# monoamine11231/Example-GUI-OpenCL-Raytracer

Hardware: AMD Instinct MI355X
Metric: Mrays/s at 1920x1080 depth 4, aggregate over n_gpus; rays = path segments + shadow rays as the reference casts them (value_traced: only those the kernel really traces) (higher is better)
Workload: dtype f32; 1 GPU; C2: scenes/render.map (regenerated), camera raypng.c:17-21, 1920x1080, depth 4, 2 soft-shadow samples, 4x256^2 textures + 4096x3072 skybox (procedural); frame=1920x1080, arithmetic=fast

## Files before the change

### example_gui_opencl_raytracer_amd/csrc/hip_wrap.cpp

```cpp
#include <hip/hip_runtime.h>

#include <algorithm>
#include <cstdarg>
#include <cstdint>
#include <cstdio>
#include <cstdlib>
#include <cmath>
#include <cstring>
#include <string>
#include <vector>

#include "../../include/hip_wrap_ext.h"
#include "png_codec.h"
#include "scene_prep.h"
#include "whitted_params.h"

extern "C" hipError_t wt_fast_launch_trace(const whitted_params*, int, unsigned, size_t, hipStream_t);
extern "C" hipError_t wt_fast_launch_raygen(const raygen_params*, hipStream_t);
extern "C" hipError_t wt_strict_launch_trace(const whitted_params*, int, unsigned, size_t, hipStream_t);
extern "C" hipError_t wt_strict_launch_raygen(const raygen_params*, hipStream_t);
extern "C" hipError_t wt_fast_launch_unit(int, const float*, float*, unsigned, unsigned, unsigned, unsigned, hipStream_t);
extern "C" hipError_t wt_strict_launch_unit(int, const float*, float*, unsigned, unsigned, unsigned, unsigned, hipStream_t);
extern "C" hipError_t wt_fast_launch_unit_scene(const whitted_params*, int, int, const float*, float*, unsigned, unsigned, unsigned, size_t, hipStream_t);
extern "C" hipError_t wt_strict_launch_unit_scene(const whitted_params*, int, int, const float*, float*, unsigned, unsigned, unsigned, size_t, hipStream_t);
// ... 364 lines not shown
            HIP_OK(hipMalloc((void**)&I->d_grid_box, bx.size() * 4), "Couldn't allocate device memory");
            HIP_OK(hipMemcpy(I->d_grid_start, st.data(), st.size() * 4, hipMemcpyHostToDevice), "Couldn't transfer the data from host to the device");
            HIP_OK(hipMemcpy(I->d_grid_items, it.data(), it.size() * 4, hipMemcpyHostToDevice), "Couldn't transfer the data from host to the device");
            HIP_OK(hipMemcpy(I->d_grid_box, bx.data(), bx.size() * 4, hipMemcpyHostToDevice), "Couldn't transfer the data from host to the device");
            std::vector<float> cg(4 * it.size(), 0.0f);
            for (size_t k = 0; k < pairs; k++) memcpy(&cg[4 * k], &geom[4 * (size_t)it[k]], 16);
            HIP_OK(hipMalloc((void**)&I->d_grid_geom, cg.size() * 4), "Couldn't allocate device memory");
            HIP_OK(hipMemcpy(I->d_grid_geom, cg.data(), cg.size() * 4, hipMemcpyHostToDevice), "Couldn't transfer the data from host to the device");
            I->grid_ok = true;
        }
    }
    I->geom_f4 = f4;
    I->scene_generation++;
    I->prep_s = s; I->prep_p = p; I->prep_l = l; I->prep_ns = ns; I->prep_np = np; I->prep_nl = nl;
}

Buffer* buffer_arg(cl_wrap* w, cl_uint kernel_id, cl_uint arg) {
    if (!is_registered(w, kernel_id, arg)) die("Couldn't run the kernel");
    return (Buffer*)w->buffers[kernel_id][arg];
}

void bind_scene(cl_wrap* w, Impl* I, cl_uint kid, whitted_params& P, int& flags, size_t& dyn_lds) {
    Kernel& k = I->kernels[kid];
    Buffer* bs = buffer_arg(w, kid, 1);
    Buffer* bp = buffer_arg(w, kid, 2);
    Buffer* bl = buffer_arg(w, kid, 3);
    uint32_t ns = read_count(k, 4), np = read_count(k, 5), nl = read_count(k, 6);
    Buffer* tex = buffer_arg(w, kid, 8);
    Buffer* sky = buffer_arg(w, kid, 9);
    if (!tex->image || !sky->image) die("Couldn't run the kernel");
    prepare_scene(I, bs, ns, bp, np, bl, nl);
    ensure_allocated(I, bs); ensure_allocated(I, bp);
    P.geom = I->d_geom; P.ptex = I->d_ptex; P.geom_f4 = (uint32_t)I->geom_f4;
    P.lpt = (I->have_lpt && !(I->variant & 128)) ? 1u : 0u;
    P.vis = (I->strict && ns <= VIS_MAX_SPHERES && (np == 0 || P.lpt) && !(I->variant & 256)) ? ((I->variant & 1024) ? 2u : 1u) : 0u;
    P.spheres_raw = (const uint8_t*)bs->dptr; P.planes_raw = (const uint8_t*)bp->dptr;
    P.ns = ns; P.np = np; P.nl = nl;
    P.through = I->through;
    P.tex = (const uint32_t*)tex->dptr; P.tex_w = (int)tex->w; P.tex_h = (int)tex->h; P.tex_layers = (int)tex->layers;
    P.sky = (const uint32_t*)sky->dptr; P.sky_w = (int)sky->w; P.sky_h = (int)sky->h;
    if (I->grid_ok && I->use_grid && !(I->variant & 8)) {
        flags |= F_GRID;
        P.grid_pair = I->grid_pair ? 1u : 0u;
        P.grid_start = I->d_grid_start; P.grid_items = I->d_grid_items; P.grid_box = I->d_grid_box; P.grid_geom = I->d_grid_geom;
        for (int a = 0; a < 3; a++) {
            P.grid_min[a] = I->grid.gmin[a]; P.grid_inv[a] = I->grid.inv[a]; P.grid_cell[a] = I->grid.cell[a]; P.grid_res[a] = I->grid.res[a];
        }
    } else if (I->geom_f4 <= GEOM_LDS_MAX_F4 && ns <= GRID_MIN_SPHERES && !(I->variant & 1)) {
        flags |= F_GEOM_LDS;
        dyn_lds = I->geom_f4 * 16;
    }
}

struct Strip { uint32_t row0, rows; int slot; };

void run_raytracer(cl_wrap* w, Impl* I, cl_uint kid, size_t array_size, const Strip* strip = nullptr) {
    Kernel& k = I->kernels[kid];
    Buffer* rays = nullptr;
    if (is_registered(w, kid, 0)) rays = (Buffer*)w->buffers[kid][0];
    else {
        const ArgValue& v = need_value(k, 0, sizeof(cl_mem), sizeof(cl_mem));
        void* h; memcpy(&h, v.bytes, sizeof h);
        rays = lookup_handle(I, h);
        if (!rays) die("Couldn't run the kernel");
    }
    uint32_t total; memcpy(&total, need_value(k, 7, 4, 4).bytes, 4);
    Buffer* out = buffer_arg(w, kid, 10);

    uint64_t rounded = ((uint64_t)array_size + BLOCK - 1) / BLOCK * BLOCK;
    uint64_t n64 = rounded < total ? rounded : total;
    ensure_allocated(I, out);
    if (n64 > out->size / 4) n64 = out->size / 4;
    if (n64 == 0) return;
    if (n64 > 0xFFFFFFFFull) die("Couldn't run the kernel");

    whitted_params P{};
    int flags = 0;
    size_t dyn_lds = 0;
    bind_scene(w, I, kid, P, flags, dyn_lds);
    P.n_items = (uint32_t)n64;
    P.depth = I->depth;
    P.out = (uint32_t*)out->dptr;
    P.out_rgb = I->debug_rgb;
    P.diag = (I->variant & 512) ? (env_int("CLWRAP_TIMELINE_EDGES", 0) ? 255u + (uint32_t)env_int("CLWRAP_TIMELINE_EDGES", 0) : 1u + (uint32_t)env_int("CLWRAP_TIMELINE_SHIFT", 0)) : 0u;

    const bool fused = I->fuse && rays->gen_valid && !rays->exposed;
    RaygenArgs g{};
    if (fused) {
        g = rays->gen;
        if (strip) {
            g.id_offset += (uint64_t)strip->row0 * g.width;
            g.n_items = strip->rows * g.width;
            P.n_items = g.n_items;
            P.out = (uint32_t*)out->dptr + (size_t)strip->row0 * g.width;
        }
        memcpy(P.corner, g.corner, 12); memcpy(P.origin, g.origin, 12);
        memcpy(P.up, g.up, 12); memcpy(P.right, g.right, 12);
        P.w_factor = g.w_factor; P.h_factor = g.h_factor; P.width = g.width; P.height = g.height;
        P.id_offset = g.id_offset;
        P.band_stride = g.band_stride; P.band_phase = g.band_phase;
        if (P.n_items > g.n_items) P.n_items = g.n_items;
        if (P.n_items == 0) return;
        P.tiled = (g.id_offset % g.width == 0 || g.band_stride > 1) && (P.n_items % g.width == 0) && !(I->variant & 2);
        P.rows = P.n_items / g.width;
        P.row_offset = (uint32_t)(g.id_offset / g.width);
        P.unit_dirs = P.ns <= GRID_MIN_SPHERES ? 1u : 0u;
    } else {
        materialise_rays(I, rays);
        ensure_allocated(I, rays);
        if ((uint64_t)P.n_items * 64 > rays->size) die("Couldn't run the kernel");
        P.rays = (const float*)rays->dptr;
        P.id_offset = I->id_offset;
        P.width = 1; P.height = 1;
        P.unit_dirs = (rays->gen_valid && !rays->exposed && P.ns <= GRID_MIN_SPHERES) ? 1u : 0u;
        if (rays->gen_valid) {
            P.id_offset = rays->gen.id_offset; P.width = rays->gen.width; P.height = rays->gen.height;
            P.band_stride = rays->gen.band_stride; P.band_phase = rays->gen.band_phase;
        } else if (I->band_stride > 1) die("Row bands need a raygen launch");
        flags |= F_RAYS;
    }
    if (I->depth > SHALLOW_LEVELS + 1) flags |= F_DEEP;
    if (!(flags & F_GEOM_LDS)) P.vis = 0;
    if (I->counting || I->stamps || I->tpt_clock) {
        if (I->counting) flags |= F_COUNT;
        P.tpt_clock = I->tpt_clock ? 1u : 0u;
        if (!I->d_counters) {
            HIP_OK(hipMalloc((void**)&I->d_counters, COUNTER_WORDS * sizeof(unsigned long long)), "Couldn't allocate device memory");
            HIP_OK(hipMemsetAsync(I->d_counters, 0, COUNTER_WORDS * sizeof(unsigned long long), I->stream), "Couldn't allocate device memory");
        }
        P.counters = I->d_counters;
    }
    unsigned grid;
    Impl::Sched& S = I->scheds[strip ? strip->slot : 0];
    bool sched_rebuild = false;
    unsigned trows = 0, tpr = 0, per_share = 0, per_share_cap = 0, base_grid = 0;
    if (P.tiled) {
        trows = (P.rows + 7) / 8; tpr = (P.width + 7) / 8;
        per_share = ((trows + 7) / 8) * tpr;
        per_share_cap = per_share;
        grid = base_grid = 8 * per_share;
    } else {
        grid = base_grid = (P.n_items + TRACE_BLOCK - 1) / TRACE_BLOCK;
    }
    if ((flags & F_DEEP) && !I->strict && (uint64_t)base_grid >= (uint64_t)I->occ_tiles_per_depth * (unsigned)I->depth && !(I->variant & 64)) flags |= F_OCC;
    const uint64_t tpt_per_node = (I->strict ? 29u : 27u) + (I->strict ? 4u : 1u) * (uint64_t)P.nl;
    const uint64_t tpt_fixed = (25u + 36u) * 64u + (uint64_t)I->depth * 3u * 64u;
    const uint64_t tpt_nslots = 8u * (uint64_t)TPT_SLOTS_PER_XCC;
    const uint64_t tpt_slice = std::min<uint64_t>(TPT_SLICE_WORDS_MAX, ((uint64_t)I->tpt_pool_mb << 18) / tpt_nslots) & ~(uint64_t)63;
    const uint64_t tpt_cap = std::min<uint64_t>(tpt_slice > tpt_fixed ? ((tpt_slice - tpt_fixed) / tpt_per_node) & ~(uint64_t)63 : 0, 64960u);
    const bool tail_wanted = (flags & F_DEEP) && !(flags & F_OCC) && !(I->variant & 16) && I->tpt_max != 0u && tpt_cap >= TPT_MIN_CAP;
    bool split = false;
    if (P.tiled) {
        if (I->sched && !(I->variant & 4) && trows <= 0xFFFu && tpr <= 0xFFFu) {
            split = tail_wanted && !(flags & F_GRID) && I->split_min_quota != 0u && !(I->variant & 4096);
            if (split) { per_share_cap = per_share + SPLIT_EXTRA_PER_SHARE; grid = 8 * per_share_cap; }
            P.cost_sum = (tail_wanted && !(flags & F_GRID)) ? 1u : 0u;
            if (S.w != P.width || S.rows != P.rows || S.cap != per_share_cap || !S.cost[0]) {
                S.free_all();
                for (int i = 0; i < 2; i++) {
                    HIP_OK(hipMalloc((void**)&S.cost[i], (size_t)trows * tpr * 4), "Couldn't allocate device memory");
                    HIP_OK(hipMalloc((void**)&S.order[i], (size_t)grid * 4), "Couldn't allocate device memory");
                    HIP_OK(hipEventCreateWithFlags(&S.built[i], hipEventDisableTiming), "Couldn't create a timing event");
                }
                HIP_OK(hipEventCreateWithFlags(&S.traced, hipEventDisableTiming), "Couldn't create a timing event");
                S.w = P.width; S.rows = P.rows; S.cap = per_share_cap; S.wr = 0;
            }
// ... 500 lines not shown
```

### example_gui_opencl_raytracer_amd/csrc/whitted_hit.inc

```
            cost++;
            if (COUNT) {
                c_iter++;
                unsigned long long live = __builtin_amdgcn_ballot_w64(true);
                if (lane == (unsigned)__builtin_ctzll(live)) c_witer += 64u;
            }
            const rayq r = UNIT_CT ? wt_rayq<true>(o, d) : wt_rayq<false>(o, d, P.unit_dirs != 0u);

            if (COUNT) c_probe++;
            bool lit = false;
            float tl = INFINITY;
            f3 lcol = mk3(0, 0, 0);
            auto probe_chunk = [&](auto nc, const unsigned base) {
                constexpr int N = decltype(nc)::value;
                float4 l0[N]; float bq[N], Dq[N]; bool ok[N]; bool any = false;
#pragma unroll
                for (int k = 0; k < N; k++) l0[k] = wt_geom<GEOM_LDS>(P, sg, g_lgt + 2 * (base + k));
#pragma unroll
                for (int k = 0; k < N; k++) {
                    const sph_pre pre = wt_sphere_pre(r.o, l0[k]);
                    ok[k] = wt_sphere_disc(pre, r.d, r.a4, bq[k], Dq[k]);
                    any |= ok[k];
                }
                if (__builtin_amdgcn_ballot_w64(any)) {
#pragma unroll
                    for (int k = 0; k < N; k++) {
                        float t;
                        const bool hit = wt_sphere_root(bq[k], Dq[k], r.a2, t) && ok[k];
                        if (hit && !(t >= tl)) {
                            float4 l1 = wt_geom<GEOM_LDS>(P, sg, g_lgt + 2 * (base + k) + 1);
                            tl = t;
                            f3 hp = wt_madd3(d, t, o);
                            float dist = wt_sqrt(dot3(o - hp, o - hp));
                            lcol = mk3(l1.x, l1.y, l1.z) * (1 / dist * dist);
                            lit = true;
                        }
                    }
                }
            };
            for (unsigned base = 0; base < SH::nl(P); base += 4u) {
                const unsigned left = SH::nl(P) - base;
                if (left >= 4u) probe_chunk(wt_int<4>{}, base);
                else if (left == 3u) probe_chunk(wt_int<3>{}, base);
                else if (left == 2u) probe_chunk(wt_int<2>{}, base);
                else probe_chunk(wt_int<1>{}, base);
            }
            if (__builtin_amdgcn_ballot_w64(lit)) {
                if (lit) {
                    if (GRID) {
                        if (wt_grid_occluded(P, r, tl)) lit = false;
                    }
                    for (unsigned i = 0; !GRID && i < SH::ns(P); i++) {
                        float4 s = wt_geom<GEOM_LDS>(P, sg, i);
                        float t;
                        bool hit = wt_sphere(r, s, t);
                        if (hit && t <= tl && !(__float_as_uint(s.w) >> 31)) lit = false;
                    }
                    for (unsigned i = 0; i < SH::np(P); i++) {
                        float4 n = wt_geom<GEOM_LDS>(P, sg, g_pln + 2 * i);
                        float4 p0 = wt_geom<GEOM_LDS>(P, sg, g_pln + 2 * i + 1);
                        float t;
                        bool hit = wt_plane(r, n, p0, t);
                        if (hit && t <= tl) lit = false;
                    }
                }
            }
            WT_STAMP(WT_ST_PROBE);
            if (lit) {
                WT_HIT_COLOUR(lcol);
                ended = true;
            } else {
                if (COUNT) c_seg++;
                float tbest = INFINITY;
                int best = -1;
                if (GRID) {
                    best = wt_grid_nearest(P, r, tbest);
                } else {
                    for (unsigned base = 0; base < SH::ns(P); base += 4u) {
                        float4 s4[4]; float bq[4], Dq[4]; bool ok[4]; bool any = false;
#pragma unroll
                        for (int k = 0; k < 4; k++) s4[k] = wt_geom<GEOM_LDS>(P, sg, min(base + k, SH::ns(P) - 1u));
#pragma unroll
                        for (int k = 0; k < 4; k++) {
                            const sph_pre pre = wt_sphere_pre(r.o, s4[k]);
                            ok[k] = wt_sphere_disc(pre, r.d, r.a4, bq[k], Dq[k]) && (base + k < SH::ns(P));
                            any |= ok[k];
                        }
                        if (__builtin_amdgcn_ballot_w64(any)) {
#pragma unroll
                            for (int k = 0; k < 4; k++) {
                                if (__builtin_amdgcn_ballot_w64(ok[k]) == 0) continue;
                                float t;
                                const bool hit = wt_sphere_root(bq[k], Dq[k], r.a2, t) && ok[k];
                                if (hit && !(t >= tbest)) { tbest = t; best = (int)(base + k); }
                            }
                        }
                    }
                }
                for (unsigned i = 0; i < SH::np(P); i++) {
                    float4 n = wt_geom<GEOM_LDS>(P, sg, g_pln + 2 * i);
                    float4 p0 = wt_geom<GEOM_LDS>(P, sg, g_pln + 2 * i + 1);
                    float t;
                    bool hit = wt_plane(r, n, p0, t);
                    if (hit && !(t >= tbest)) { tbest = t; best = (int)(SH::ns(P) + i); }
                }
                WT_STAMP(WT_ST_NEAREST);
                if (best < 0) {
                    if (COUNT) c_sky++;
                    WT_HIT_COLOUR(wt_texel_rgb(wt_skybox_fetch(P, d)));
                    ended = true;
                } else {
                    ip = wt_madd3(d, tbest, o);
                    prim = (unsigned)best;
                    textured = false;
                    if ((unsigned)best < SH::ns(P)) {
                        float4 s = wt_geom<GEOM_LDS>(P, sg, (unsigned)best);
                        nrm = wt_normalize(ip - mk3(s.x, s.y, s.z));
                    } else {
                        unsigned pi = (unsigned)best - SH::ns(P);
                        float4 n = wt_geom<GEOM_LDS>(P, sg, g_pln + 2 * pi);
                        nrm = mk3(n.x, n.y, n.z);
                        if (n.w != 0.0f) {
                            if (COUNT) c_tex++;
                            texpx = wt_plane_texel_fetch(P, pi, ip);
                            textured = true;
                        }
                    }
                    wt_mat_set_b(m, wt_mat_f4(P, prim, 1u, SH::ns(P)));
                    {
                        const float4 a_ = wt_mat_f4(P, prim, 0u, SH::ns(P));
                        m.rgb = mk3(a_.x, a_.y, a_.z);
                        wt_mat_set_c(m, wt_mat_f4(P, prim, 2u, SH::ns(P)));
                    }
                    ip = wt_madd3(nrm, WT_EPSILON, ip);
                    cost += 3u;
                    {
                        const f3 c_ = textured ? wt_texel_rgb(texpx) : m.rgb;
                        WT_HIT_AMBIENT(c_ * f, m.ambient);
                    }
                    view = wt_normalize(o - ip);
                    ks = f * m.specular; kd = f * m.diffuse;
                    shade = true;
                }
            }
```

### example_gui_opencl_raytracer_amd/csrc/whitted_params.h

```cpp
#ifndef WHITTED_PARAMS_H
#define WHITTED_PARAMS_H
#include <stdint.h>

#define CLW_MAX_DEPTH 32
#define CLW_NUM_COUNTERS 32
#define CLW_STAMP_SHARDS 1024

typedef struct {
    float corner[3], origin[3], up[3], right[3];
    float w_factor, h_factor;
    uint32_t width, height;
    uint64_t id_offset;
    uint32_t n_items;
    uint32_t tiled;
    uint32_t rows;
    uint32_t row_offset;
    uint32_t band_stride, band_phase;
    const uint32_t* tile_order;
    uint32_t* tile_cost;
    uint32_t* tpt_pool;
    uint32_t* tpt_flags;
    const uint32_t* tpt_jump;
    uint32_t tpt_slice_words, tpt_cap, tpt_slots, tpt_max, tpt_min;
    uint32_t tpt_clock;
    uint32_t cost_sum;
    int32_t depth;
    const float* geom;
    const float* ptex;
    const uint8_t* spheres_raw;
    const uint8_t* planes_raw;
    uint32_t ns, np, nl;
    float through;
    uint32_t geom_f4;
    uint32_t unit_dirs;
    uint32_t lpt;
    uint32_t vis;
    uint32_t diag;
    const uint32_t* grid_start;
    const uint32_t* grid_items;
    const uint32_t* grid_box;
    const float* grid_geom;
    float grid_min[3], grid_inv[3], grid_cell[3];
    uint32_t grid_pair;
    int32_t grid_res[3];
    const uint32_t* tex; int32_t tex_w, tex_h, tex_layers;
    const uint32_t* sky; int32_t sky_w, sky_h;
    const float* rays;
    uint32_t* out;
    float* out_rgb;
    unsigned long long* counters;
} whitted_params;

typedef struct {
    float corner[3], origin[3], up[3], right[3];
    float w_factor, h_factor;
    uint32_t width, height;
    uint64_t id_offset;
    uint32_t n_items;
    uint32_t band_stride, band_phase;
    float* rays;
} raygen_params;

#endif
```

### example_gui_opencl_raytracer_amd/csrc/whitted_trace.inc

```

#ifndef WT_STRICT
#error "WT_STRICT must be defined (0: fast, 1: strict)"
#endif

#define WT_EPSILON 0.001f
#define WT_THROUGH 0.8f
#define WT_DEFAULT_N 1.0f
#define WT_SOFT 2
#ifndef WT_LDS_LEVELS
#if WT_STRICT
#define WT_LDS_LEVELS 3
#else
#define WT_LDS_LEVELS 2
#endif
#endif
#ifndef WT_LDS_LEVELS_DEEP
#define WT_LDS_LEVELS_DEEP 3
#endif
#ifndef WT_LDS_LEVELS_DEEP_OCC
#define WT_LDS_LEVELS_DEEP_OCC 1
#endif
#ifndef WT_MIN_WAVES
#define WT_MIN_WAVES (WT_STRICT ? 2 : 3)
#endif
// ... 898 lines not shown
    typedef wt_shape<SHF> SH;
    const bool masked = MASKED && P.ns <= 64u;
    unsigned long long todo = !masked ? 0ull : ((P.ns == 64u ? ~0ull : ((1ull << P.ns) - 1ull)) & cand);
    for (unsigned n = 0; todo != 0ull; n++) {
        const unsigned i = (unsigned)__builtin_ctzll(todo);
        todo &= todo - 1ull;
        if ((n & 3u) == 3u) {
            unsigned live = 0u;
#pragma unroll
            for (int q = 0; q < NR; q++) live |= __float_as_uint(op[q]);
            if (__builtin_amdgcn_ballot_w64(live != 0u) == 0) break;
        }
        const float4 s = wt_geom<GEOM_LDS>(P, sg, i);
        const sph_pre pre = wt_shadow_pre(ip, s);
        const float through = (__float_as_uint(s.w) >> 31) ? P.through : 0.0f;
        float bq[NR], Dq[NR];
        bool any = false;
#pragma unroll
        for (int q = 0; q < NR; q++) any |= wt_shadow_disc_g<GEOM_LDS>(pre, rd[q], a4[q], bq[q], Dq[q]);
        if (__builtin_amdgcn_ballot_w64(any)) {
#pragma unroll
            for (int q = 0; q < NR; q++) {
                float t;
                bool hit = wt_shadow_root_g<GEOM_LDS>(bq[q], Dq[q], a2[q], t) && !(Dq[q] < 0);
                if (hit && !(t >= tl[q])) op[q] = op[q] * through;
            }
        }
    }
    for (unsigned i = 0; !masked && i < SH::ns(P); i++) {
        if ((i & 3u) == 3u) {
            unsigned live = 0u;
#pragma unroll
            for (int q = 0; q < NR; q++) live |= __float_as_uint(op[q]);
            if (__builtin_amdgcn_ballot_w64(live != 0u) == 0) break;
        }
        const float4 s = wt_geom<GEOM_LDS>(P, sg, i);
        const sph_pre pre = wt_shadow_pre(ip, s);
        const float through = (__float_as_uint(s.w) >> 31) ? P.through : 0.0f;
        float bq[NR], Dq[NR];
        bool any = false;
#pragma unroll
        for (int q = 0; q < NR; q++) any |= wt_shadow_disc_g<GEOM_LDS>(pre, rd[q], a4[q], bq[q], Dq[q]);
        if (__builtin_amdgcn_ballot_w64(any)) {
#pragma unroll
            for (int q = 0; q < NR; q++) {
                float t;
                bool hit = wt_shadow_root_g<GEOM_LDS>(bq[q], Dq[q], a2[q], t) && !(Dq[q] < 0);
                if (hit && !(t >= tl[q])) op[q] = op[q] * through;
            }
        }
    }
    for (unsigned i = 0; i < SH::np(P); i++) {
        if ((i & 3u) == 0u) {
            unsigned live = 0u;
#pragma unroll
            for (int q = 0; q < NR; q++) live |= __float_as_uint(op[q]);
            if (__builtin_amdgcn_ballot_w64(live != 0u) == 0) break;
        }
        const float4 n = wt_geom<GEOM_LDS>(P, sg, g_pln + 2 * i);
        const float4 p0 = wt_geom<GEOM_LDS>(P, sg, g_pln + 2 * i + 1);
        const float num = wt_plane_pre(ip, n, p0);
        bool skip[NR / WT_SOFT];
#pragma unroll
        for (int k = 0; k < NR / WT_SOFT; k++) skip[k] = false;
        if (CULL && SH::lpt(P) && chunk != ~0u) {
            const float4 mu = wt_geom<GEOM_LDS>(P, sg, g_pln + 2 * SH::np(P) + 2 * SH::nl(P) + chunk * SH::np(P) + i);
            const float mus[3] = {mu.x, mu.y, mu.z};
            const float an = 1e-5f * fabsf(num) * mu.w;
#pragma unroll
            for (int k = 0; k < NR / WT_SOFT && k < 3; k++) {
                const bool cannot = (num * mus[k] < 0.0f) && (fabsf(mus[k]) > __builtin_fmaf(4e-6f, dlc[k], an));
                skip[k] = __builtin_amdgcn_ballot_w64(!cannot) == 0;
            }
        }
#pragma unroll
        for (int q = 0; q < NR; q++) {
            if (!skip[q / WT_SOFT]) {
                if (wt_plane_blocks(num, n, rd[q], tl[q])) op[q] = 0.0f;
            }
        }
    }
}

__device__ __forceinline__ void wt_stage_scene(const whitted_params& P, float4* s_geom, unsigned tid, unsigned nthreads) {
    for (unsigned i = tid; i < P.geom_f4; i += nthreads) s_geom[i] = ((const float4*)P.geom)[i];
    __syncthreads();
}

#include "whitted_terms.inc"

template <int FLAGS>
struct wt_cfg {
    static constexpr bool deep = (FLAGS & 2) != 0, occ = (FLAGS & 32) != 0, grid = (FLAGS & 16) != 0;
    static constexpr int lds_levels = deep ? (occ ? WT_LDS_LEVELS_DEEP_OCC : WT_LDS_LEVELS_DEEP) : WT_LDS_LEVELS;
    static constexpr int max_levels = !deep ? 3 : ((FLAGS & 64) ? 7 : ((FLAGS & 128) ? 15 : CLW_MAX_DEPTH - 1));
    static constexpr int min_waves = deep ? (occ ? WT_OCC_WAVES : WT_MIN_WAVES) : ((grid && !WT_STRICT) ? WT_GRID_SHALLOW_WAVES : WT_SHALLOW_WAVES);
};
typedef const __attribute__((address_space(4))) whitted_params* wt_kparams_t;
template <int FLAGS>
__device__ __forceinline__ void wt_trace_body(const wt_kparams_t Pk, const unsigned wg) {
    constexpr bool COUNT = (FLAGS & WT_F_COUNT) != 0;
    constexpr bool DEEP = (FLAGS & WT_F_DEEP) != 0;
    constexpr bool GEOM_LDS = (FLAGS & WT_F_GEOM_LDS) != 0;
    constexpr bool FROM_RAYS = (FLAGS & WT_F_RAYS) != 0;
    constexpr bool GRID = (FLAGS & WT_F_GRID) != 0;
    constexpr bool UNIT_CT = !WT_STRICT && GEOM_LDS && !FROM_RAYS && !GRID;
    constexpr bool CLASSES = WT_STRICT != 0 && GEOM_LDS && !GRID;

    constexpr int LDSL = wt_cfg<FLAGS>::lds_levels;
    __shared__ float s_stk[LDSL * WT_REC * WT_BLOCK];
    __shared__ unsigned short s_tpt_bs[(DEEP && !wt_cfg<FLAGS>::occ) ? WT_TPT_MAX_BATCHES + 2 : 1];
    __shared__ unsigned s_tpt_px[(DEEP && !wt_cfg<FLAGS>::occ) ? 3 * 64 : 1];
    constexpr bool SPHCULL = DEEP && !GRID && (wt_cfg<FLAGS>::occ || WT_STRICT != 0);
    __shared__ int s_cull[SPHCULL ? 8 : 1];
    extern __shared__ float4 s_geom[];

    const whitted_params& P = *(const whitted_params*)Pk;
#if WT_TIMELINE
    const unsigned long long tl_entry = __builtin_amdgcn_s_memrealtime();
#endif

    if (GEOM_LDS) wt_stage_scene(P, s_geom, threadIdx.x, WT_BLOCK);
    const float4* sg = s_geom;
#if WT_TIMELINE
    const unsigned long long tl_staged = __builtin_amdgcn_s_memrealtime();
#endif
    WT_STAMP_DECL

    const unsigned tid = threadIdx.x;
    const unsigned lane = tid & 63u;

    bool valid;
    unsigned item;
    unsigned x = 0, y = 0;
    unsigned tile = 0xFFFFFFFFu;
    unsigned part_lg = 0u, part = 0u;
    if (P.tiled) {
        const unsigned tpr = (P.width + 7u) >> 3;
        const unsigned b = wg;
        unsigned trow, tcol;
        if (P.tile_order) {
            const unsigned t = P.tile_order[b];
            tcol = t & 0xFFFu; trow = (t >> 12) & 0xFFFu;
            part_lg = (t >> 24) & 7u; part = (t >> 27) & 15u;
            tile = (t == 0xFFFFFFFFu) ? t : trow * tpr + tcol;
        } else {
            const unsigned k = b & 7u, j = b >> 3;
            trow = (j / tpr) * 8u + k;
            tcol = j % tpr;
            tile = trow * tpr + tcol;
        }
        x = tcol * 8u + (lane & 7u);
        y = trow * 8u + (lane >> 3);
        valid = (tile != 0xFFFFFFFFu) && (x < P.width) && (y < P.rows) && ((lane >> (6u - part_lg)) == part);
        item = y * P.width + x;
    } else {
        item = wg * WT_BLOCK + tid;
        valid = item < P.n_items;
        if (P.band_stride > 1u) { y = item / P.width; x = item % P.width; }
    }
#if WT_TIMELINE
    asm volatile("" :: "v"(item), "v"(x), "v"(y));
    const unsigned long long tl_mapped = __builtin_amdgcn_s_memrealtime();
#endif
    unsigned long long gid = P.id_offset + item;
    unsigned gy = y;
    if (P.band_stride > 1u) {
        gy = ((y >> 3) * P.band_stride + P.band_phase) * 8u + (y & 7u);
        gid = (unsigned long long)gy * P.width + x;
    } else if (P.tiled) {
        gy = P.row_offset + y;
    }

    constexpr int SCRL = wt_cfg<FLAGS>::max_levels - LDSL;
    float deep[SCRL > 0 ? SCRL * WT_REC : 1];

    f3 o = mk3(0, 0, 0), d = mk3(0, 0, 1), rgb = mk3(0, 0, 0);
    int depth = 0;
    if (valid) {
        if (FROM_RAYS) {
            const float4* rr = (const float4*)(P.rays + 16 * (size_t)item);
            float4 ro = rr[0], rd = rr[1], rc = rr[2];
            o = mk3(ro.x, ro.y, ro.z); d = mk3(rd.x, rd.y, rd.z); rgb = mk3(rc.x, rc.y, rc.z);
            depth = __float_as_int(rr[3].x);
        } else {
            if (P.tiled || P.band_stride > 1u) d = wt_primary_dir_xy(P.corner, P.right, P.up, P.w_factor, P.h_factor, x, gy);
            else d = wt_primary_dir(P.corner, P.right, P.up, P.w_factor, P.h_factor, (unsigned)gid, P.width);
            o = mk3(P.origin[0], P.origin[1], P.origin[2]);
        }
    }
    float n1 = WT_DEFAULT_N, f = 1.0f;
    int sp = 0;
    unsigned rng = (unsigned)gid;
    const int D = P.depth;
    bool active = valid && depth < D;

    unsigned c_seg = 0, c_shadow = 0, c_probe = 0, c_sky = 0, c_tex = 0, c_push = 0, c_iter = 0, c_witer = 0;
    unsigned c_traced = 0;
    unsigned c_known = 0, c_visbad = 0;
    unsigned c_tptrun = 0, c_tptfail = 0, c_tptnodes = 0;

    typedef wt_shape<FLAGS> SH;
    const unsigned g_pln = SH::ns(P), g_lgt = SH::ns(P) + 2 * SH::np(P);

    const unsigned long long t_begin = ((GRID || WT_COST_LIFETIME) && P.tile_cost) ? __builtin_amdgcn_s_memtime() : 0ull;
#if WT_TIMELINE
    const unsigned long long tl_begin = __builtin_amdgcn_s_memrealtime();
    unsigned long long tl_end = tl_begin;
#endif
    unsigned cost = 0;
#ifndef WT_LCH
#define WT_LCH 3
#endif
    constexpr int LCH = WT_LCH, NR = LCH * WT_SOFT;

    constexpr bool TPT = DEEP && !wt_cfg<FLAGS>::occ;
    unsigned tpt_thresh = (TPT && P.tpt_cap != 0u) ? (part_lg != 0u ? 64u : P.tpt_max) : 0u;
    WT_STAMP(WT_ST_PROLOG);
    for (;;) {
    while ((unsigned)__builtin_popcountll(__builtin_amdgcn_ballot_w64(active)) > tpt_thresh) {
        if (active) {
            WT_STAMP(WT_ST_LOOP);
            bool ended = false, shade = false;
            f3 ip, nrm, view;
            mat_t m;
            float ks, kd;
            unsigned prim, texpx;
            bool textured;
#include "whitted_hit.inc"
            WT_STAMP(WT_ST_RESOLVE);
            if (shade) {
#include "whitted_shade.inc"
#include "whitted_bounce.inc"
            WT_STAMP(WT_ST_BOUNCE);
            }
#include "whitted_pop.inc"
            WT_STAMP(WT_ST_POP);
        }
    }
    if (!TPT || __builtin_amdgcn_ballot_w64(active) == 0) break;
    {
        bool tpt_done = false;
#include "whitted_tpt.inc"
        if (tpt_done) break;
        tpt_thresh = 0u;
    }
    }
    if (P.tiled && P.tile_cost) {
        unsigned c = cost;
        if (GRID || WT_COST_LIFETIME) c = (unsigned)min((__builtin_amdgcn_s_memtime() - t_begin) >> 8, 0xFFFFFFFFull);
        else if (P.cost_sum) for (int off = 32; off > 0; off >>= 1) c += (unsigned)__shfl_xor((int)c, off);
        else for (int off = 32; off > 0; off >>= 1) c = max(c, (unsigned)__shfl_xor((int)c, off));
#if WT_TIMELINE
        if (P.diag && P.diag < 256u) c = ((unsigned)((tl_begin >> (P.diag - 1u)) & 0xFFFFull) << 16) | (unsigned)((__builtin_amdgcn_s_memrealtime() >> (P.diag - 1u)) & 0xFFFFull);
        tl_end = __builtin_amdgcn_s_memrealtime();
#endif
        if (lane == 0 && tile != 0xFFFFFFFFu && y < P.rows) {
            if (P.cost_sum && !(WT_TIMELINE && P.diag)) atomicAdd(P.tile_cost + tile, c);
            else P.tile_cost[tile] = c;
        }
    }


    if (valid) {
        if (P.out_rgb) {
            float* q = P.out_rgb + 3 * (size_t)item;
            q[0] = rgb.x; q[1] = rgb.y; q[2] = rgb.z;
        }
        float cr = fminf(fmaxf(rgb.x, 0.0f), 1.0f) * 255.0f;
        float cg = fminf(fmaxf(rgb.y, 0.0f), 1.0f) * 255.0f;
        float cb = fminf(fmaxf(rgb.z, 0.0f), 1.0f) * 255.0f;
        P.out[item] = ((unsigned)cr << 16) | ((unsigned)cg << 8) | (unsigned)cb;
    }

#ifdef WT_STAMPS
    WT_STAMP(WT_ST_LOOP);
    __syncthreads();
    if (P.counters && lane == 0) {
        unsigned long long* sh = P.counters + CLW_NUM_COUNTERS + 16u * (wg & 1023u);
        for (int k = 0; k < WT_ST_N; k++) atomicAdd(sh + k, (unsigned long long)s_st[k]);
        atomicAdd(sh + WT_ST_N, 1ull);
    }
#endif
    if (COUNT) {
        unsigned v[14] = {c_seg, c_shadow, c_probe, c_sky, c_tex, c_push, c_iter, c_witer, c_traced, c_known, c_visbad, c_tptfail, c_tptrun, c_tptnodes};
#pragma unroll
        for (int k = 0; k < 14; k++) {
            unsigned x = v[k];
            for (int off = 32; off > 0; off >>= 1) x += __shfl_xor(x, off);
            if (lane == 0 && x) atomicAdd(P.counters + (k < 10 ? k : 18 + k), (unsigned long long)x);
        }
    }
#if WT_TIMELINE
    if (P.diag >= 256u && P.tiled && P.tile_cost && lane == 0 && tile != 0xFFFFFFFFu && y < P.rows) {
        __builtin_amdgcn_s_waitcnt(0);
        if (P.diag == 256u) P.tile_cost[tile] = ((unsigned)min(tl_begin - tl_entry, 0xFFFFull) << 16) | (unsigned)min(__builtin_amdgcn_s_memrealtime() - tl_end, 0xFFFFull);
        else P.tile_cost[tile] = ((unsigned)min(tl_staged - tl_entry, 1023ull) << 22) | ((unsigned)min(tl_mapped - tl_staged, 2047ull) << 11) | (unsigned)min(tl_begin - tl_mapped, 2047ull);
    }
#endif
}
template <int FLAGS>
__global__ void __launch_bounds__(WT_BLOCK, wt_cfg<FLAGS>::min_waves) wt_trace(const whitted_params P_arg) {
    const wt_kparams_t Pk = (wt_kparams_t)__builtin_amdgcn_kernarg_segment_ptr();
    wt_trace_body<FLAGS>(Pk, blockIdx.x);
}

#define WT_RG_BLOCK 256
__global__ void __launch_bounds__(WT_RG_BLOCK) wt_raygen(const raygen_params P) {
    constexpr int RS = WT_RG_BLOCK + 1;
    __shared__ float4 s_rec[4 * RS];
    const unsigned tid = threadIdx.x;
    const size_t base = (size_t)blockIdx.x * WT_RG_BLOCK;
    const size_t item = base + tid;
    float4 r0 = make_float4(0, 0, 0, 0), r1 = r0;
    if (item < P.n_items) {
        unsigned long long gid = P.id_offset + item;
        if (P.band_stride > 1u) {
            const unsigned y = (unsigned)(item / P.width), x = (unsigned)(item % P.width);
            gid = (unsigned long long)(((y >> 3) * P.band_stride + P.band_phase) * 8u + (y & 7u)) * P.width + x;
        }
        f3 d = wt_primary_dir(P.corner, P.right, P.up, P.w_factor, P.h_factor, (unsigned)gid, P.width);
        r0 = make_float4(P.origin[0], P.origin[1], P.origin[2], 0.0f);
        r1 = make_float4(d.x, d.y, d.z, 0.0f);
    }
    s_rec[0 * RS + tid] = r0;
    s_rec[1 * RS + tid] = r1;
    s_rec[2 * RS + tid] = make_float4(0, 0, 0, 0);
    s_rec[3 * RS + tid] = make_float4(0, 0, 0, 0);
    __syncthreads();
    float4* dst = (float4*)P.rays + base * 4;
    const size_t limit = ((size_t)P.n_items - base < WT_RG_BLOCK ? (size_t)P.n_items - base : WT_RG_BLOCK) * 4;
#pragma unroll
    for (int k = 0; k < 4; k++) {
        size_t q = (size_t)k * WT_RG_BLOCK + tid;
        if (q < limit) dst[q] = s_rec[(q & 3) * RS + (q >> 2)];
    }
}

__global__ void __launch_bounds__(256) wt_sched_build(const unsigned* __restrict__ cost, unsigned* __restrict__ order,
                                                      unsigned tpr, unsigned trows, unsigned per_share, unsigned clamp_outliers,
                                                      unsigned per_share_cap, unsigned split_slots, unsigned min_quota) {
    __shared__ unsigned hist[256];
    __shared__ unsigned base[256];
    __shared__ unsigned s_max, s_cnt, s_entries;
    __shared__ unsigned long long s_sum;
    const unsigned k = blockIdx.x, tid = threadIdx.x;
    hist[tid] = 0;
    if (tid == 0) { s_max = 1u; s_cnt = 0u; s_sum = 0ull; s_entries = 0u; }
    __syncthreads();
    unsigned cnt = 0u;
    unsigned long long sum = 0ull;
    for (unsigned j = tid; j < per_share; j += 256) {
        const unsigned trow = (j / tpr) * 8u + k;
        if (trow < trows) { sum += cost[trow * tpr + (j % tpr)]; cnt++; }
    }
    atomicAdd(&s_sum, sum); atomicAdd(&s_cnt, cnt);
    __syncthreads();
    unsigned quota = 0xFFFFFFFFu;
    if (split_slots != 0u) {
        const unsigned long long q = s_sum / split_slots;
        quota = (unsigned)(q > 0x7FFFFFFFull ? 0x7FFFFFFFull : q);
        if (quota < min_quota) quota = min_quota;
        if (quota == 0u) quota = 1u;
        for (int trial = 0; trial < 24; trial++) {
            if (tid == 0) s_entries = 0u;
            __syncthreads();
            unsigned e = 0u;
            for (unsigned j = tid; j < per_share; j += 256) {
                const unsigned trow = (j / tpr) * 8u + k;
                if (trow < trows) { unsigned lg = 0u; const unsigned c = cost[trow * tpr + (j % tpr)]; while (lg < 4u && (c >> lg) > quota) lg++; e += 1u << lg; }
            }
            atomicAdd(&s_entries, e);
            __syncthreads();
// ... 43 lines not shown
    for (unsigned j = nvalid + tid; j < per_share_cap; j += 256) order[8u * j + k] = 0xFFFFFFFFu;
}

enum { WT_U_SPHERE = 0, WT_U_PLANE = 1, WT_U_REFLECT = 2, WT_U_REFRACT = 3, WT_U_SCHLICK = 4, WT_U_CUBE = 5,
       WT_U_XORSHIFT = 6, WT_U_EMOD = 7, WT_U_SINCOS = 8, WT_U_POW = 9, WT_U_NORMALIZE = 10 };
__global__ void __launch_bounds__(64) wt_unit(int op, const float* __restrict__ in, float* __restrict__ out, unsigned n,
                                              unsigned stride_in, unsigned stride_out, unsigned aux) {
    const unsigned i = blockIdx.x * 64 + threadIdx.x;
    if (i >= n) return;
    const float* a = in + (size_t)i * stride_in;
    float* r = out + (size_t)i * stride_out;
    switch (op) {
        case WT_U_SPHERE: {
            const rayq q = wt_rayq<false>(mk3(a[0], a[1], a[2]), mk3(a[3], a[4], a[5]));
            float t;
            bool hit = wt_sphere(q, make_float4(a[6], a[7], a[8], a[9] * a[9]), t);
            r[0] = hit ? 1.0f : 0.0f; r[1] = hit ? t : 0.0f;
        } break;
        case WT_U_PLANE: {
            const rayq q = wt_rayq<false>(mk3(a[0], a[1], a[2]), mk3(a[3], a[4], a[5]));
            float t;
            bool hit = wt_plane(q, make_float4(a[6], a[7], a[8], 0.0f), make_float4(a[9], a[10], a[11], 0.0f), t);
            r[0] = hit ? 1.0f : 0.0f; r[1] = hit ? t : 0.0f;
        } break;
        case WT_U_REFLECT: {
            f3 v = wt_reflect(mk3(a[0], a[1], a[2]), mk3(a[3], a[4], a[5]));
            r[0] = v.x; r[1] = v.y; r[2] = v.z;
        } break;
        case WT_U_REFRACT: {
            f3 v = mk3(0, 0, 0);
            bool ok = wt_refract(a[0], a[1], mk3(a[2], a[3], a[4]), mk3(a[5], a[6], a[7]), v);
            r[0] = ok ? 1.0f : 0.0f; r[1] = v.x; r[2] = v.y; r[3] = v.z;
        } break;
        case WT_U_SCHLICK:
            r[0] = wt_schlick(a[0], a[1], mk3(a[2], a[3], a[4]), mk3(a[5], a[6], a[7]));
            break;
        case WT_U_CUBE: {
            int u, v;
            wt_cube_uv(mk3(a[0], a[1], a[2]), aux, u, v);
            r[0] = __int_as_float(u); r[1] = __int_as_float(v);
        } break;
        case WT_U_XORSHIFT: {
            unsigned st = __float_as_uint(a[0]);
            float v = wt_xorshift(st);
            r[0] = __uint_as_float(st); r[1] = v;
        } break;
        case WT_U_EMOD:
            r[0] = __int_as_float(wt_emod(__float_as_int(a[0]), __float_as_int(a[1])));
            break;
        case WT_U_SINCOS: {
            float sn, cs;
            if (aux) wt_sincos_angle<true>(a[0], sn, cs); else wt_sincos_angle<false>(a[0], sn, cs);
            r[0] = sn; r[1] = cs;
        } break;
        case WT_U_POW:
            r[0] = wt_pow(a[0], a[1]);
            break;
        case WT_U_NORMALIZE: {
            float len;
            f3 v = wt_normalize_len(mk3(a[0], a[1], a[2]), len);
            r[0] = v.x; r[1] = v.y; r[2] = v.z; r[3] = len;
        } break;
        default: break;
    }
}

enum { WT_US_HIT = 0, WT_US_SHADOW = 1, WT_US_TEXEL = 2 };
template <bool GEOM_LDS, bool GRID>
__global__ void __launch_bounds__(64) wt_unit_scene(const whitted_params P, int op, const float* __restrict__ in,
                                                    float* __restrict__ out, unsigned n, unsigned stride_in, unsigned stride_out) {
    extern __shared__ float4 s_geom[];
    const unsigned tid = threadIdx.x, lane = tid & 63u;
    constexpr bool UNIT_CT = false;
    if (GEOM_LDS) wt_stage_scene(P, s_geom, tid, 64u);
    const float4* sg = s_geom;
    typedef wt_shape<0> SH;
    const unsigned g_pln = P.ns, g_lgt = P.ns + 2 * P.np;
    const unsigned i = blockIdx.x * 64 + tid;
    if (i >= n) return;
    const float* a = in + (size_t)i * stride_in;
    float* res = out + (size_t)i * stride_out;
    WT_STAMP_DECL
    constexpr bool COUNT = false, FROM_RAYS = false;
    unsigned cost = 0, c_iter = 0, c_witer = 0, c_probe = 0, c_seg = 0, c_sky = 0, c_tex = 0;
    (void)lane; (void)c_iter; (void)c_witer; (void)c_probe; (void)c_seg; (void)c_sky; (void)c_tex;
    if (op == WT_US_HIT) {
        f3 o = mk3(a[0], a[1], a[2]), d = mk3(a[3], a[4], a[5]), rgb = mk3(0, 0, 0);
        const float f = 1.0f;
        bool ended = false, shade = false;
        f3 ip = mk3(0, 0, 0), nrm = mk3(0, 0, 0), view = mk3(0, 0, 0);
        mat_t m;
        m.rgb = mk3(0, 0, 0); m.ambient = m.diffuse = m.specular = m.shininess = 0.0f;
        m.transparent = m.dielectric = 0u; m.n = 0.0f; m.reflectivity = 0.0f;
        float ks = 0.0f, kd = 0.0f;
        unsigned prim = 0u, texpx = 0u;
        bool textured = false;
        {
#include "whitted_hit.inc"
            res[0] = lit ? 1.0f : 0.0f;
            if (lit) { res[1] = rgb.x; res[2] = rgb.y; res[3] = rgb.z; }
        }
        (void)ended; (void)view; (void)ks; (void)kd; (void)cost;
        res[4] = shade ? 1.0f : 0.0f;
        if (shade) {
            if (textured) m.rgb = wt_texel_rgb(texpx);
            res[5] = ip.x; res[6] = ip.y; res[7] = ip.z; res[8] = nrm.x; res[9] = nrm.y; res[10] = nrm.z;
            res[11] = m.rgb.x; res[12] = m.rgb.y; res[13] = m.rgb.z; res[14] = m.ambient; res[15] = m.diffuse; res[16] = m.specular;
            res[17] = m.shininess; res[18] = (float)m.transparent; res[19] = (float)m.dielectric; res[20] = m.n; res[21] = m.reflectivity;
        }
    } else if (op == WT_US_SHADOW) {
        const f3 to = mk3(a[0], a[1], a[2]), from = mk3(a[3], a[4], a[5]);
        constexpr int NR = WT_SOFT * 3;
        f3 rd[NR]; float tl[NR], a4[NR], a2[NR], opq[NR];
#pragma unroll
        for (int q = 0; q < NR; q++) { rd[q] = mk3(0, 0, 0); tl[q] = 0.0f; a4[q] = 0.0f; a2[q] = 0.0f; opq[q] = 0.0f; }
        rd[0] = wt_normalize_len(to - from, tl[0]);
        const rayq rq = wt_shadow_rayq_scene<GEOM_LDS>(P, from, rd[0]);
        a4[0] = rq.a4; a2[0] = rq.a2; opq[0] = 1.0f;
        if (GRID) {
            opq[0] = wt_grid_shadow(P, from, rd[0], rq.a4, rq.a2, tl[0]);
            for (unsigned k = 0; k < P.np; k++) {
                const float4 pn = wt_geom<GEOM_LDS>(P, sg, g_pln + 2 * k);
                const float4 p0 = wt_geom<GEOM_LDS>(P, sg, g_pln + 2 * k + 1);
                if (wt_plane_blocks(wt_plane_pre(from, pn, p0), pn, rd[0], tl[0])) opq[0] = 0.0f;
            }
        } else {
            const float dlc[NR / WT_SOFT] = {0.0f, 0.0f, 0.0f};
            wt_shadow_batch<GEOM_LDS, NR, false>(P, sg, g_pln, from, rd, tl, a4, a2, opq, ~0u, dlc);
        }
        res[0] = opq[0];
    } else if (op == WT_US_TEXEL) {
        whitted_params Q = P;
        Q.ptex = a;
        const f3 c = wt_texel_rgb(wt_plane_texel_fetch(Q, 0u, mk3(a[8], a[9], a[10])));
        res[0] = c.x; res[1] = c.y; res[2] = c.z;
    }
}
```

Before: 345,400 Mrays/s.

## Add per-wavefront cone culling of primary-ray primitives in tiled trace

Builds a conservative cone around each 64-lane tile's primary ray directions. One lane per primitive tests whether each sphere, light or plane can be hit by any ray in the cone, and a ballot produces a cull mask. On the first bounce, intersection tests for culled primitives are skipped, and the mask is reset to all-ones after that iteration. A counting mode records when a culled primitive would actually have been hit, to validate the cone bounds. It only applies to non-grid, LDS-staged, shape-specialized kernels, and it adds setup cost per wave plus a risk of wrong images if the bounds are not conservative enough.

```diff
diff --git a/example_gui_opencl_raytracer_amd/csrc/hip_wrap.cpp b/example_gui_opencl_raytracer_amd/csrc/hip_wrap.cpp
--- a/example_gui_opencl_raytracer_amd/csrc/hip_wrap.cpp
+++ b/example_gui_opencl_raytracer_amd/csrc/hip_wrap.cpp
@@ -470,6 +470,7 @@
     P.depth = I->depth;
     P.out = (uint32_t*)out->dptr;
     P.out_rgb = I->debug_rgb;
+    P.cull = (I->variant & 16384) ? 0u : (I->counting ? 2u : 1u);
     P.diag = (I->variant & 512) ? (env_int("CLWRAP_TIMELINE_EDGES", 0) ? 255u + (uint32_t)env_int("CLWRAP_TIMELINE_EDGES", 0) : 1u + (uint32_t)env_int("CLWRAP_TIMELINE_SHIFT", 0)) : 0u;
 
     const bool fused = I->fuse && rays->gen_valid && !rays->exposed;
diff --git a/example_gui_opencl_raytracer_amd/csrc/whitted_hit.inc b/example_gui_opencl_raytracer_amd/csrc/whitted_hit.inc
--- a/example_gui_opencl_raytracer_amd/csrc/whitted_hit.inc
+++ b/example_gui_opencl_raytracer_amd/csrc/whitted_hit.inc
@@ -17,6 +17,7 @@
                 for (int k = 0; k < N; k++) l0[k] = wt_geom<GEOM_LDS>(P, sg, g_lgt + 2 * (base + k));
 #pragma unroll
                 for (int k = 0; k < N; k++) {
+                    if (CULL_T == 1 && !wt_cbit(cullm, base + k)) { ok[k] = false; bq[k] = 0.0f; Dq[k] = 0.0f; continue; }
                     const sph_pre pre = wt_sphere_pre(r.o, l0[k]);
                     ok[k] = wt_sphere_disc(pre, r.d, r.a4, bq[k], Dq[k]);
                     any |= ok[k];
@@ -26,6 +27,7 @@
                     for (int k = 0; k < N; k++) {
                         float t;
                         const bool hit = wt_sphere_root(bq[k], Dq[k], r.a2, t) && ok[k];
+                        if (CULL_T == 2 && hit && !wt_cbit(cullm, base + k)) c_cullbad++;
                         if (hit && !(t >= tl)) {
                             float4 l1 = wt_geom<GEOM_LDS>(P, sg, g_lgt + 2 * (base + k) + 1);
                             tl = t;
@@ -81,6 +83,7 @@
                         for (int k = 0; k < 4; k++) s4[k] = wt_geom<GEOM_LDS>(P, sg, min(base + k, SH::ns(P) - 1u));
 #pragma unroll
                         for (int k = 0; k < 4; k++) {
+                            if (CULL_T == 1 && !wt_cbit(cullm, SH::nl(P) + base + k)) { ok[k] = false; bq[k] = 0.0f; Dq[k] = 0.0f; continue; }
                             const sph_pre pre = wt_sphere_pre(r.o, s4[k]);
                             ok[k] = wt_sphere_disc(pre, r.d, r.a4, bq[k], Dq[k]) && (base + k < SH::ns(P));
                             any |= ok[k];
@@ -91,16 +94,20 @@
                                 if (__builtin_amdgcn_ballot_w64(ok[k]) == 0) continue;
                                 float t;
                                 const bool hit = wt_sphere_root(bq[k], Dq[k], r.a2, t) && ok[k];
+                                if (CULL_T == 2 && hit && !wt_cbit(cullm, SH::nl(P) + base + k)) c_cullbad++;
                                 if (hit && !(t >= tbest)) { tbest = t; best = (int)(base + k); }
                             }
                         }
                     }
                 }
                 for (unsigned i = 0; i < SH::np(P); i++) {
+                    const bool tst = wt_cbit(cullm, SH::nl(P) + SH::ns(P) + i);
+                    if (CULL_T == 1 && !tst) continue;
                     float4 n = wt_geom<GEOM_LDS>(P, sg, g_pln + 2 * i);
                     float4 p0 = wt_geom<GEOM_LDS>(P, sg, g_pln + 2 * i + 1);
                     float t;
                     bool hit = wt_plane(r, n, p0, t);
+                    if (CULL_T == 2 && hit && !tst) c_cullbad++;
                     if (hit && !(t >= tbest)) { tbest = t; best = (int)(SH::ns(P) + i); }
                 }
                 WT_STAMP(WT_ST_NEAREST);
diff --git a/example_gui_opencl_raytracer_amd/csrc/whitted_params.h b/example_gui_opencl_raytracer_amd/csrc/whitted_params.h
--- a/example_gui_opencl_raytracer_amd/csrc/whitted_params.h
+++ b/example_gui_opencl_raytracer_amd/csrc/whitted_params.h
@@ -36,6 +36,7 @@
     uint32_t lpt;
     uint32_t vis;
     uint32_t diag;
+    uint32_t cull;
     const uint32_t* grid_start;
     const uint32_t* grid_items;
     const uint32_t* grid_box;
diff --git a/example_gui_opencl_raytracer_amd/csrc/whitted_trace.inc b/example_gui_opencl_raytracer_amd/csrc/whitted_trace.inc
--- a/example_gui_opencl_raytracer_amd/csrc/whitted_trace.inc
+++ b/example_gui_opencl_raytracer_amd/csrc/whitted_trace.inc
@@ -1004,6 +1004,36 @@
     }
 }
 
+__device__ __forceinline__ bool wt_cbit(unsigned long long m, unsigned i) { return i >= 64u || ((m >> i) & 1ull) != 0ull; }
+__device__ __forceinline__ unsigned long long wt_tile_cull(const whitted_params& P, const float4* sg, unsigned ns, unsigned np, unsigned nl,
+                                                           f3 d, bool active, unsigned lane) {
+    auto rl = [](float v, int l) { return __int_as_float(__builtin_amdgcn_readlane(__float_as_int(v), l)); };
+    const f3 o = mk3(P.origin[0], P.origin[1], P.origin[2]);
+    const f3 ax = mk3(rl(d.x, 27), rl(d.y, 27), rl(d.z, 27));
+    const float c = dot3(d, ax);
+    const float ct = fminf(fminf(rl(c, 0), rl(c, 7)), fminf(rl(c, 56), rl(c, 63))) - 4e-6f;
+    if (__builtin_amdgcn_ballot_w64(active && !(c >= ct)) != 0ull || !(ct > 0.2f)) return ~0ull;
+    const float cm = ct - 2e-6f;
+    const float st = __builtin_amdgcn_sqrtf(__builtin_fmaf(-cm, cm, 1.0f));
+    bool clear = false;
+    if (lane < nl + ns) {
+        const float4 s = sg[lane < nl ? ns + 2u * np + 2u * lane : lane - nl];
+        const f3 w = mk3(s.x, s.y, s.z) - o;
+        const float ww = dot3(w, w), sx = dot3(w, ax);
+        const float p2 = __builtin_fmaf(-sx, sx, ww);
+        const float t1 = __builtin_fmaf(sx, st, __builtin_fmaf(4e-3f, __builtin_amdgcn_sqrtf(ww), __builtin_amdgcn_sqrtf(fabsf(s.w)))) * 1.0001f;
+        clear = t1 < 0.0f || p2 * (cm * cm) > t1 * t1;
+    } else if (lane < nl + ns + np) {
+        const unsigned i = lane - nl - ns;
+        const float4 n = sg[ns + 2u * i], p0 = sg[ns + 2u * i + 1u];
+        const float num = wt_plane_pre(o, n, p0);
+        const f3 n3 = mk3(n.x, n.y, n.z);
+        const float an = dot3(ax, n3), lim = (st + 2e-4f) * __builtin_amdgcn_sqrtf(dot3(n3, n3)) * 1.0001f;
+        clear = (num > 0.0f && an < -lim) || (num < 0.0f && an > lim);
+    }
+    return ~__builtin_amdgcn_ballot_w64(clear);
+}
+
 __device__ __forceinline__ void wt_stage_scene(const whitted_params& P, float4* s_geom, unsigned tid, unsigned nthreads) {
     for (unsigned i = tid; i < P.geom_f4; i += nthreads) s_geom[i] = ((const float4*)P.geom)[i];
     __syncthreads();
@@ -1124,6 +1154,12 @@
 
     typedef wt_shape<FLAGS> SH;
     const unsigned g_pln = SH::ns(P), g_lgt = SH::ns(P) + 2 * SH::np(P);
+
+    constexpr int CULL_T = (!WT_STRICT && GEOM_LDS && !FROM_RAYS && !GRID && !DEEP) ? (((FLAGS & WT_F_SHAPE) != 0) ? 1 : (COUNT ? 2 : 0)) : 0;
+    unsigned long long cullm = ~0ull;
+    unsigned c_cullbad = 0;
+    if (CULL_T != 0 && P.cull == (unsigned)CULL_T && P.tiled) cullm = wt_tile_cull(P, sg, SH::ns(P), SH::np(P), SH::nl(P), d, active, lane);
+    const bool c_cullw = CULL_T == 2 && cullm != ~0ull;
 
     const unsigned long long t_begin = ((GRID || WT_COST_LIFETIME) && P.tile_cost) ? __builtin_amdgcn_s_memtime() : 0ull;
 #if WT_TIMELINE
@@ -1159,6 +1195,7 @@
 #include "whitted_pop.inc"
             WT_STAMP(WT_ST_POP);
         }
+        if (CULL_T != 0) cullm = ~0ull;
     }
     if (!TPT || __builtin_amdgcn_ballot_w64(active) == 0) break;
     {
@@ -1211,6 +1248,12 @@
             unsigned x = v[k];
             for (int off = 32; off > 0; off >>= 1) x += __shfl_xor(x, off);
             if (lane == 0 && x) atomicAdd(P.counters + (k < 10 ? k : 18 + k), (unsigned long long)x);
+        }
+        if (CULL_T == 2) {
+            unsigned x = c_cullbad;
+            for (int off = 32; off > 0; off >>= 1) x += __shfl_xor(x, off);
+            if (lane == 0 && x) atomicAdd(P.counters + 27, (unsigned long long)x);
+            if (lane == 0 && c_cullw) atomicAdd(P.counters + 26, 1ull);
         }
     }
 #if WT_TIMELINE
@@ -1420,6 +1463,10 @@
     float* res = out + (size_t)i * stride_out;
     WT_STAMP_DECL
     constexpr bool COUNT = false, FROM_RAYS = false;
+    constexpr int CULL_T = 0;
+    const unsigned long long cullm = ~0ull;
+    unsigned c_cullbad = 0;
+    (void)cullm; (void)c_cullbad;
     unsigned cost = 0, c_iter = 0, c_witer = 0, c_probe = 0, c_seg = 0, c_sky = 0, c_tex = 0;
     (void)lane; (void)c_iter; (void)c_witer; (void)c_probe; (void)c_seg; (void)c_sky; (void)c_tex;
     if (op == WT_US_HIT) {
```

After: 325,600 Mrays/s (median of 2 runs). -5.7%, worse.
